# NVIDIA/tacotron2

Measured on AMD Instinct MI355X. Metric: mel-frames/sec (train fwd+bwd) LJSpeech hparams, higher is better.
Workload: dtype bf16; 1 GPU; BASELINE configs[1]: LJSpeech default hparams, batch_size=64/GPU, synthetic LJSpeech-shaped batches, full train step (fwd+loss+bwd+clip+Adam); global_batch=64, parallelism=dp1, optimizer=FusedAdam, compute=bf16 MFMA operands, f32 accumulate/state/master weights

## Files before the change

### include/tacotron2_amd.h

```cpp
#ifndef TACOTRON2_AMD_H
#define TACOTRON2_AMD_H

#include <stdint.h>

#ifdef __cplusplus
extern "C" {
#endif

#define T2AMD_ABI_VERSION 1
#define T2AMD_OK 0
#define T2AMD_ERR_ARG 1
#define T2AMD_ERR_LAUNCH 2

#define T2AMD_ATT_DIM 128
#define T2AMD_LOC_FILTERS 32
#define T2AMD_LOC_KERNEL 31
#define T2AMD_LOC_TAPS (2 * T2AMD_LOC_KERNEL)
#define T2AMD_ATT_SLICES 4

int t2amd_abi_version(void);
const char* t2amd_source_sha1(void);
const char* t2amd_last_error(void);
int t2amd_struct_sizes(int* out, int max_n);
int t2amd_set_validate_only(int on);
// ... 3 lines not shown

typedef struct t2amd_gemm_desc {
    const float* A;
    const float* B;
    float* C;
    int M, N, K;
    long long lda, ldb, ldc;
    int a_kcontig;
    int b_kcontig;
    int batch;
    long long strideA, strideB, strideC;
    int splitk;
    long long strideSplitC;
    int accumulate;
    const float* bias;
    int act;
    const uint8_t* keep;
    long long ldkeep;
    float keep_scale;
    int convA_T, convA_C, convA_pad, convA_sign;
    int convB_T, convB_C, convB_pad;
    int precision;
} t2amd_gemm_desc;

int t2amd_gemm_tile_size(int M, int N, int precision, int nz, int a_kcontig, int b_kcontig);
int t2amd_gemm_f32(const t2amd_gemm_desc* d, void* stream);

int t2amd_splitk_reduce_f32(const float* partials, int nsplit, long long stride, float* out,
                            long long n, int accumulate, int perm_taps, int perm_ci, void* stream);
int t2amd_splitk_reduce2d_f32(const float* partials, int nsplit, long long stride, float* out, int rows, int cols,
                              long long ldo, int accumulate, void* stream);

typedef struct t2amd_gemm16_desc {
    const void* A;
    const void* B;
    float* C;
    int M, N, K;
    long long lda, ldb, ldc;
    int splitk;
    long long strideSplitC;
    int accumulate;
    const float* bias;
    int win_T, win_Tp;
} t2amd_gemm16_desc;
int t2amd_gemm16_tn(const t2amd_gemm16_desc* d, void* stream);
int t2amd_gemm16_kk(const t2amd_gemm16_desc* d, void* stream);
// ... 653 lines not shown
```

### tacotron2_amd/csrc/attention.hip

```cpp
#include "common.h"
#include "cell_bwd.h"
#include "skinny_wide.h"
#include <vector>
#include <cstring>
#include <stdlib.h>
#include <stddef.h>

__device__ unsigned int t2_attn_timeouts = 0u;
__device__ __forceinline__ void t2_attn_gave_up() { atomicAdd(&t2_attn_timeouts, 1u); }
extern "C" int t2amd_attn_handoff_timeouts(int reset) {
    if (t2amd_validate_only_flag_()) return 0;
    unsigned int v = 0u;
    if (hipMemcpyFromSymbol(&v, HIP_SYMBOL(t2_attn_timeouts), sizeof(v)) != hipSuccess) return -1;
    if (reset && v != 0u) {
        const unsigned int z = 0u;
        (void)hipMemcpyToSymbol(HIP_SYMBOL(t2_attn_timeouts), &z, sizeof(z));
    }
    return (int)(v > 0x7fffffffu ? 0x7fffffffu : v);
}
__global__ void t2_attn_bump_kernel() { t2_attn_gave_up(); }
extern "C" int t2amd_debug_attn_timeout_(void* stream) {
    hipLaunchKernelGGL(t2_attn_bump_kernel, dim3(1), dim3(1), 0, (hipStream_t)stream);
    return hipGetLastError() == hipSuccess ? 0 : -1;
}
// ... 2435 lines not shown
extern "C" int t2amd_attention_step_bwd_f32(const t2amd_attn_bwd* a, void* stream) {
    return attn_bwd_step_impl(a, stream);
}


__global__ void fold_location_kernel(const float* __restrict__ wd, const float* __restrict__ wc,
                                     float* __restrict__ U) {
    const int i = blockIdx.x * blockDim.x + threadIdx.x;
    if (i < AD * NTAP) {
        const int d = i / NTAP, ck = i - d * NTAP;
        float s = 0.f;
        for (int f = 0; f < T2AMD_LOC_FILTERS; ++f) s = fmaf(wd[d * T2AMD_LOC_FILTERS + f], wc[f * NTAP + ck], s);
        U[i] = s;
    }
}

extern "C" int t2amd_fold_location_f32(const float* wdense, const float* wconv, float* U, void* stream) {
    T2_REQUIRE(wdense && wconv && U && t2_aligned16(U), "fold_location: bad pointers");
    T2_LAUNCH(fold_location_kernel, dim3((AD * NTAP + 255) / 256), dim3(256), 0, (hipStream_t)stream, wdense, wconv, U);
    T2_LAUNCH_CHECK();
    return T2AMD_OK;
}

__global__ __launch_bounds__(256) void unfold_location_reduce_kernel(const float* __restrict__ dU_acc, const float* __restrict__ dv_acc,
                                                                     int nb, float* __restrict__ dv, float* __restrict__ dUsum) {
    const int i = blockIdx.x * 256 + threadIdx.x;
    if (i < AD * NTAP) {
        float s = 0.f;
        int b = 0;
        for (; b + 8 <= nb; b += 8) {
            float v[8];
#pragma unroll
            for (int j = 0; j < 8; ++j) v[j] = dU_acc[(long long)(b + j) * AD * NTAP + i];
#pragma unroll
            for (int j = 0; j < 8; ++j) s += v[j];
        }
        for (; b < nb; ++b) s += dU_acc[(long long)b * AD * NTAP + i];
        dUsum[i] = s;
    } else if (i < AD * NTAP + AD) {
        const int d = i - AD * NTAP;
        float s = 0.f;
        for (int b = 0; b < nb; ++b) s += dv_acc[(long long)b * AD + d];
        dv[d] = s;
    }
}
__global__ __launch_bounds__(256) void unfold_location_products_kernel(const float* __restrict__ dUsum, const float* __restrict__ wd,
                                                                       const float* __restrict__ wc, float* __restrict__ dwd,
                                                                       float* __restrict__ dwc) {
    const int i = blockIdx.x * 256 + threadIdx.x;
    if (i < AD * T2AMD_LOC_FILTERS) {
        const int d = i / T2AMD_LOC_FILTERS, f = i - d * T2AMD_LOC_FILTERS;
        float s = 0.f;
        for (int ck = 0; ck < NTAP; ++ck) s = fmaf(dUsum[d * NTAP + ck], wc[f * NTAP + ck], s);
        dwd[i] = s;
    } else if (i < AD * T2AMD_LOC_FILTERS + T2AMD_LOC_FILTERS * NTAP) {
        const int o = i - AD * T2AMD_LOC_FILTERS;
        const int f = o / NTAP, ck = o - f * NTAP;
        float s = 0.f;
        for (int d = 0; d < AD; ++d) s = fmaf(wd[d * T2AMD_LOC_FILTERS + f], dUsum[d * NTAP + ck], s);
        dwc[o] = s;
    }
}

extern "C" int t2amd_unfold_location_grads_f32(const float* dU_acc, const float* dv_acc, int nb,
                                               const float* wdense, const float* wconv, float* dwdense,
                                               float* dwconv, float* dv, void* stream) {
    T2_REQUIRE(dU_acc && dv_acc && nb > 0 && wdense && wconv && dwdense && dwconv && dv, "unfold_location: bad args");
    float* dUsum = const_cast<float*>(dU_acc);
    T2_LAUNCH(unfold_location_reduce_kernel, dim3(t2_cdiv(AD * NTAP + AD, 256)), dim3(256), 0, (hipStream_t)stream, dU_acc, dv_acc, nb,
              dv, dUsum);
    T2_LAUNCH(unfold_location_products_kernel, dim3(t2_cdiv(AD * T2AMD_LOC_FILTERS + T2AMD_LOC_FILTERS * NTAP, 256)), dim3(256), 0,
              (hipStream_t)stream, dUsum, wdense, wconv, dwdense, dwconv);
    T2_LAUNCH_CHECK();
    return T2AMD_OK;
}
```

### tacotron2_amd/csrc/gemm.hip

```cpp
#include "common.h"

#define GBM 128
#define GBN 128
#define GBK 16
#define GLD 132

struct GemmParams {
    t2amd_gemm_desc d;
    int avec, bvec;
    int ktiles_per_split;
};

struct TileId { int bx, by, bz; };
__device__ __forceinline__ TileId xcd_tile_id() {
    const int nbx = gridDim.x, nby = gridDim.y;
    const int total = nbx * nby * (int)gridDim.z;
    const int L = blockIdx.x + nbx * (blockIdx.y + nby * blockIdx.z);
    const int xcd = L & 7, q = L >> 3;
    const int base = total >> 3, rem = total & 7;
    const int id = xcd * base + (xcd < rem ? xcd : rem) + q;
    const int per_z = nbx * nby;
    TileId t;
    t.bz = id / per_z;
    const int r = id - t.bz * per_z;
    const int G = 8;
    const int group = r / (G * nbx);
    const int first = group * G;
    const int gsz = (nby - first) < G ? (nby - first) : G;
    const int w = r - group * (G * nbx);
    t.by = first + w % gsz;
    t.bx = w / gsz;
    return t;
}
// ... 220 lines not shown
#pragma unroll
    for (int tm = 0; tm < 2; ++tm) {
#pragma unroll
        for (int tn = 0; tn < 2; ++tn) {
            const int gn = col0 + wn * 64 + tn * 32 + l31;
#pragma unroll
            for (int r = 0; r < 16; ++r) {
                const int row = (r & 3) + 8 * (r >> 2) + 4 * lhi;
                const int gm = row0 + wm * 64 + tm * 32 + row;
                if (gm < M && gn < N) {
                    float val = acc[tm][tn][r];
                    float* cp = C + (long long)gm * d.ldc + gn;
                    if (d.bias) val += d.bias[gn];
                    if (d.accumulate) val += *cp;
                    if (d.act == 1) val = fmaxf(val, 0.f);
                    if (d.keep) val = d.keep[(long long)gm * d.ldkeep + gn] ? val * d.keep_scale : 0.f;
                    *cp = val;
                }
            }
        }
    }
}

template <bool AK, bool BKC, bool X3, int TB>
__global__ __launch_bounds__(2 * TB) void gemm_bf16x3_kernel(GemmParams p);

extern "C" int t2amd_gemm_tile_size(int M, int N, int precision, int nz, int a_kcontig, int b_kcontig) {
    static const bool force128 = [] { const char* e = getenv("T2AMD_GEMM_TILE"); return e && atoi(e) == 128; }();
    if (force128 || precision < 1 || M < 512 || N < 512) return 128;
    if (precision == 1 && (a_kcontig || b_kcontig)) return 128;
    const long long wgs = (long long)t2_cdiv(M, 256) * t2_cdiv(N, 256) * (nz > 0 ? nz : 1);
    return wgs >= 192 ? 256 : 128;
}

extern "C" int t2amd_gemm_f32(const t2amd_gemm_desc* dp, void* stream) {
    T2_REQUIRE(dp != nullptr, "gemm: null descriptor");
    GemmParams p;
    p.d = *dp;
    t2amd_gemm_desc& d = p.d;
    T2_REQUIRE(d.A && d.B && d.C, "gemm: null operand");
    T2_REQUIRE(d.M > 0 && d.N > 0 && d.K >= 0, "gemm: bad dims");
    if (d.batch < 1) d.batch = 1;
    if (d.splitk < 1) d.splitk = 1;
    if (d.convA_T > 0) {
        T2_REQUIRE(d.a_kcontig == 1, "gemm: convA needs K-contiguous A");
        T2_REQUIRE(d.convA_C % GBK == 0 && d.K % d.convA_C == 0, "gemm: convA_C must be a multiple of 16 dividing K");
        T2_REQUIRE(d.convA_sign == 1 || d.convA_sign == -1, "gemm: convA_sign must be +-1");
        T2_REQUIRE(d.M % d.convA_T == 0, "gemm: convA rows must be whole utterances");
    }
    if (d.convB_T > 0) {
        T2_REQUIRE(d.b_kcontig == 0, "gemm: convB needs N-contiguous B");
        T2_REQUIRE(d.convB_C % 4 == 0 && d.N % d.convB_C == 0, "gemm: convB_C must be a multiple of 4 dividing N");
        T2_REQUIRE(d.K % d.convB_T == 0, "gemm: convB rows must be whole utterances");
    }
    if (d.splitk > 1) {
        T2_REQUIRE(!d.bias && !d.keep && d.act == 0 && !d.accumulate, "gemm: split-K needs a plain epilogue");
    }
    T2_REQUIRE(d.act == 0 || d.act == 1, "gemm: act must be 0 or 1");
    if (d.a_kcontig) {
        const int kdim = d.convA_T > 0 ? d.convA_C : d.K;
        p.avec = (kdim % 4 == 0) && (d.lda % 4 == 0) && t2_aligned16(d.A) && (d.strideA % 4 == 0);
    } else {
        p.avec = (d.M % 4 == 0) && (d.lda % 4 == 0) && t2_aligned16(d.A) && (d.strideA % 4 == 0);
    }
    if (d.b_kcontig) {
        p.bvec = (d.K % 4 == 0) && (d.ldb % 4 == 0) && t2_aligned16(d.B) && (d.strideB % 4 == 0);
    } else {
        const int ndim = d.convB_T > 0 ? d.convB_C : d.N;
        p.bvec = (ndim % 4 == 0) && (d.ldb % 4 == 0) && t2_aligned16(d.B) && (d.strideB % 4 == 0);
    }
    T2_REQUIRE(d.precision >= 0 && d.precision <= 2, "gemm: precision must be 0 (exact f32), 1 (split-bf16 x3) or 2 (bf16)");
    const bool fast = d.precision >= 1 && (d.convA_T == 0 || d.convA_C % 32 == 0);
    const int bk = fast ? 32 : GBK;
    const int nkt = t2_cdiv(d.K, bk);
    p.ktiles_per_split = t2_cdiv(nkt > 0 ? nkt : 1, d.splitk);
    dim3 grid(t2_cdiv(d.N, GBN), t2_cdiv(d.M, GBM), d.batch * d.splitk);
    T2_REQUIRE(grid.y <= 65535 && grid.z <= 65535, "gemm: grid too large");
    hipStream_t s = (hipStream_t)stream;
    if (fast && d.precision == 1 && t2amd_gemm_tile_size(d.M, d.N, 1, d.batch * d.splitk, d.a_kcontig, d.b_kcontig) == 256) {
        dim3 g2(t2_cdiv(d.N, 256), t2_cdiv(d.M, 256), d.batch * d.splitk);
        static bool attr_set = false;
        if (!attr_set && !t2amd_validate_only_flag_()) {
            (void)hipFuncSetAttribute((const void*)gemm_bf16x3_kernel<false, false, true, 256>,
                                      hipFuncAttributeMaxDynamicSharedMemorySize, 0);
            attr_set = true;
        }
        T2_LAUNCH((gemm_bf16x3_kernel<false, false, true, 256>), g2, dim3(512), 0, s, p);
        T2_LAUNCH_CHECK();
        return T2AMD_OK;
    }
    if (fast && d.precision == 1) {
        if (d.a_kcontig && d.b_kcontig)
            T2_LAUNCH((gemm_bf16x3_kernel<true, true, true, 128>), grid, dim3(256), 0, s, p);
        else if (d.a_kcontig && !d.b_kcontig)
            T2_LAUNCH((gemm_bf16x3_kernel<true, false, true, 128>), grid, dim3(256), 0, s, p);
        else if (!d.a_kcontig && d.b_kcontig)
            T2_LAUNCH((gemm_bf16x3_kernel<false, true, true, 128>), grid, dim3(256), 0, s, p);
        else
            T2_LAUNCH((gemm_bf16x3_kernel<false, false, true, 128>), grid, dim3(256), 0, s, p);
        T2_LAUNCH_CHECK();
        return T2AMD_OK;
    }
    if (fast && d.precision == 2 && t2amd_gemm_tile_size(d.M, d.N, 2, d.batch * d.splitk, d.a_kcontig, d.b_kcontig) == 256) {
        dim3 g2(t2_cdiv(d.N, 256), t2_cdiv(d.M, 256), d.batch * d.splitk);
        if (d.a_kcontig && d.b_kcontig)
            T2_LAUNCH((gemm_bf16x3_kernel<true, true, false, 256>), g2, dim3(512), 0, s, p);
        else if (d.a_kcontig && !d.b_kcontig)
            T2_LAUNCH((gemm_bf16x3_kernel<true, false, false, 256>), g2, dim3(512), 0, s, p);
        else if (!d.a_kcontig && d.b_kcontig)
            T2_LAUNCH((gemm_bf16x3_kernel<false, true, false, 256>), g2, dim3(512), 0, s, p);
        else
            T2_LAUNCH((gemm_bf16x3_kernel<false, false, false, 256>), g2, dim3(512), 0, s, p);
        T2_LAUNCH_CHECK();
        return T2AMD_OK;
    }
    if (fast) {
        if (d.a_kcontig && d.b_kcontig)
            T2_LAUNCH((gemm_bf16x3_kernel<true, true, false, 128>), grid, dim3(256), 0, s, p);
        else if (d.a_kcontig && !d.b_kcontig)
            T2_LAUNCH((gemm_bf16x3_kernel<true, false, false, 128>), grid, dim3(256), 0, s, p);
        else if (!d.a_kcontig && d.b_kcontig)
            T2_LAUNCH((gemm_bf16x3_kernel<false, true, false, 128>), grid, dim3(256), 0, s, p);
        else
            T2_LAUNCH((gemm_bf16x3_kernel<false, false, false, 128>), grid, dim3(256), 0, s, p);
        T2_LAUNCH_CHECK();
// ... 82 lines not shown
}

typedef short bf16x8 __attribute__((ext_vector_type(8)));

#define HBM_ 128
#define HBN_ 128
#define HBK_ 32
#define HLD_ 40

__device__ __forceinline__ unsigned cvt_pk_bf16(float a, float b) {
    unsigned r;
    asm("v_cvt_pk_bf16_f32 %0, %1, %2" : "=v"(r) : "v"(a), "v"(b));
    return r;
}
__device__ __forceinline__ void split4(float x0, float x1, float x2, float x3, uint2& hi, uint2& lo) {
    hi.x = cvt_pk_bf16(x0, x1);
    hi.y = cvt_pk_bf16(x2, x3);
    const float h0 = __uint_as_float(hi.x << 16), h1 = __uint_as_float(hi.x & 0xffff0000u);
    const float h2 = __uint_as_float(hi.y << 16), h3 = __uint_as_float(hi.y & 0xffff0000u);
    lo.x = cvt_pk_bf16(x0 - h0, x1 - h1);
    lo.y = cvt_pk_bf16(x2 - h2, x3 - h3);
}

template <bool AK, bool BKC, bool X3, int TB>
__global__ __launch_bounds__(2 * TB) void gemm_bf16x3_kernel(GemmParams p) {
    constexpr int NTHR = 2 * TB;
    constexpr int WN = TB / 64;
    constexpr int TM = TB / 64;
    constexpr int NH = X3 ? 2 : 1;
    constexpr int ALD = AK ? HLD_ : 32, BLD = BKC ? HLD_ : 32;
    constexpr int AIMG = TB * ALD, BIMG = TB * BLD;
    __shared__ __attribute__((aligned(16))) unsigned short As[2][NH * AIMG];
    __shared__ __attribute__((aligned(16))) unsigned short Bs[2][NH * BIMG];

    const t2amd_gemm_desc& d = p.d;
    const int tid = threadIdx.x;
    const int lane = tid & 63;
    const int wave = tid >> 6;
    const int wm = wave / WN, wn = wave % WN;

    const TileId tile = xcd_tile_id();
    const int z = tile.bz;
    const int bidx = z / d.splitk;
    const int split = z - bidx * d.splitk;
    const float* __restrict__ A = d.A + (long long)bidx * d.strideA;
    const float* __restrict__ B = d.B + (long long)bidx * d.strideB;
    float* __restrict__ C = d.C + (long long)bidx * d.strideC + (long long)split * d.strideSplitC;

    const int row0 = tile.by * TB;
    const int col0 = tile.bx * TB;
    const int M = d.M, N = d.N;
    const int kbeg = split * p.ktiles_per_split * HBK_;
    int kend = kbeg + p.ktiles_per_split * HBK_;
    if (kend > d.K) kend = d.K;
    const int nk = (kend > kbeg) ? (kend - kbeg + HBK_ - 1) / HBK_ : 0;

    int a_t[4] = {0, 0, 0, 0};
    if (AK && d.convA_T > 0) {
#pragma unroll
        for (int i = 0; i < 4; ++i) a_t[i] = (row0 + ((tid + NTHR * i) >> 3)) % d.convA_T;
    }
    int b_tap = 0, b_ci = 0;
    if (!BKC && d.convB_T > 0) {
        const int gn = col0 + (tid & (TB / 4 - 1)) * 4;
        b_tap = gn / d.convB_C;
        b_ci = gn - b_tap * d.convB_C;
    }

    float4 ra[4], rb[4];

    auto load_a = [&](int k0) {
#pragma unroll
        for (int i = 0; i < 4; ++i) {
            float4 v = make_float4(0.f, 0.f, 0.f, 0.f);
            if (AK) {
                const int f = tid + NTHR * i;
                const int r = f >> 3, kq = f & 7;
                const int gm = row0 + r;
                const int gk = k0 + kq * 4;
                if (gm < M && gk < kend) {
                    long long srow = gm;
                    int col = gk;
                    bool ok = true;
                    if (d.convA_T > 0) {
                        const int tap = k0 / d.convA_C;
                        col = (k0 - tap * d.convA_C) + kq * 4;
                        const int sh = (tap - d.convA_pad) * d.convA_sign;
                        const int tt = a_t[i] + sh;
                        ok = (tt >= 0) && (tt < d.convA_T);
                        srow = (long long)gm + sh;
                    }
                    if (ok) {
                        const float* src = A + srow * d.lda + col;
                        if (p.avec) {
// ... 7 lines not shown
                    }
                }
            } else {
                const int m4 = tid & (TB / 4 - 1), kq = tid / (TB / 4);
                const int gk = k0 + kq * 4 + i;
                const int gm = row0 + m4 * 4;
                if (gk < kend && gm < M) {
                    const float* src = A + (long long)gk * d.lda + gm;
                    if (p.avec) {
                        v = *reinterpret_cast<const float4*>(src);
                    } else {
                        v.x = src[0];
                        if (gm + 1 < M) v.y = src[1];
                        if (gm + 2 < M) v.z = src[2];
                        if (gm + 3 < M) v.w = src[3];
                    }
                }
            }
            ra[i] = v;
        }
    };

    auto load_b = [&](int k0) {
#pragma unroll
        for (int i = 0; i < 4; ++i) {
            float4 v = make_float4(0.f, 0.f, 0.f, 0.f);
            if (BKC) {
                const int f = tid + NTHR * i;
                const int r = f >> 3, kq = f & 7;
                const int gn = col0 + r;
                const int gk = k0 + kq * 4;
                if (gn < N && gk < kend) {
                    const float* src = B + (long long)gn * d.ldb + gk;
                    if (p.bvec) {
                        v = *reinterpret_cast<const float4*>(src);
                    } else {
                        v.x = src[0];
                        if (gk + 1 < kend) v.y = src[1];
                        if (gk + 2 < kend) v.z = src[2];
                        if (gk + 3 < kend) v.w = src[3];
                    }
                }
            } else {
                const int n4 = tid & (TB / 4 - 1), kq = tid / (TB / 4);
                const int gk = k0 + kq * 4 + i;
                const int gn = col0 + n4 * 4;
// ... 76 lines not shown
        } else {
            const unsigned* P = reinterpret_cast<const unsigned*>(S);
            const int p0 = ks * 8 + lhi_ * 4;
            union { unsigned u[4]; bf16x8 v; } t;
            t.u[0] = P[(p0 + 0) * TB + row];
            t.u[1] = P[(p0 + 1) * TB + row];
            t.u[2] = P[(p0 + 2) * TB + row];
            t.u[3] = P[(p0 + 3) * TB + row];
            return t.v;
        }
    };

    f32x16 acc[TM][2];
#pragma unroll
    for (int i = 0; i < TM; ++i)
#pragma unroll
        for (int j = 0; j < 2; ++j)
#pragma unroll
            for (int r = 0; r < 16; ++r) acc[i][j][r] = 0.f;

    if (nk > 0) {
        load_a(kbeg);
        load_b(kbeg);
        store_one(As[0], AIMG, AK, ra);
        store_one(Bs[0], BIMG, BKC, rb);
    }
    __syncthreads();

    const int l31 = lane & 31, lhi = lane >> 5;
    int cur = 0;
    for (int kt = 0; kt < nk; ++kt) {
        const bool more = (kt + 1 < nk);
        if (more) {
            load_a(kbeg + (kt + 1) * HBK_);
            load_b(kbeg + (kt + 1) * HBK_);
        }
#pragma unroll
        for (int ks = 0; ks < HBK_ / 16; ++ks) {
            bf16x8 ah[TM], al[TM], bh[2], bl[2];
#pragma unroll
            for (int t = 0; t < TM; ++t) {
                ah[t] = frag(As[cur], AK, wm * (32 * TM) + t * 32 + l31, ks, lhi);
                if (X3) al[t] = frag(As[cur] + AIMG, AK, wm * (32 * TM) + t * 32 + l31, ks, lhi);
            }
#pragma unroll
            for (int t = 0; t < 2; ++t) {
                bh[t] = frag(Bs[cur], BKC, wn * 64 + t * 32 + l31, ks, lhi);
                if (X3) bl[t] = frag(Bs[cur] + BIMG, BKC, wn * 64 + t * 32 + l31, ks, lhi);
            }
#pragma unroll
            for (int i = 0; i < TM; ++i)
#pragma unroll
                for (int j = 0; j < 2; ++j) {
                    if (X3) {
                        acc[i][j] = __builtin_amdgcn_mfma_f32_32x32x16_bf16(al[i], bh[j], acc[i][j], 0, 0, 0);
                        acc[i][j] = __builtin_amdgcn_mfma_f32_32x32x16_bf16(ah[i], bl[j], acc[i][j], 0, 0, 0);
                    }
                    acc[i][j] = __builtin_amdgcn_mfma_f32_32x32x16_bf16(ah[i], bh[j], acc[i][j], 0, 0, 0);
                }
        }
        if (more) {
            store_one(As[cur ^ 1], AIMG, AK, ra);
            store_one(Bs[cur ^ 1], BIMG, BKC, rb);
        }
        __syncthreads();
        cur ^= 1;
    }

#pragma unroll
    for (int tm = 0; tm < TM; ++tm) {
#pragma unroll
        for (int tn = 0; tn < 2; ++tn) {
            const int gn = col0 + wn * 64 + tn * 32 + l31;
#pragma unroll
            for (int r = 0; r < 16; ++r) {
                const int row = (r & 3) + 8 * (r >> 2) + 4 * lhi;
                const int gm = row0 + wm * (32 * TM) + tm * 32 + row;
                if (gm < M && gn < N) {
                    float val = acc[tm][tn][r];
                    float* cp = C + (long long)gm * d.ldc + gn;
                    if (d.bias) val += d.bias[gn];
                    if (d.accumulate) val += *cp;
                    if (d.act == 1) val = fmaxf(val, 0.f);
                    if (d.keep) val = d.keep[(long long)gm * d.ldkeep + gn] ? val * d.keep_scale : 0.f;
                    *cp = val;
                }
// ... 5 lines not shown
```

### tacotron2_amd/csrc/rnn.hip

```cpp
#include "common.h"
#include "cell_bwd.h"
#include <hip/hip_ext.h>

#include "skinny_wide.h"

#define SK_DEPTH 4

template <bool LSTM, int TAG, bool BF>
__global__ __launch_bounds__(256) void skinny_gemm_kernel(SkinnyDual dp) {
    constexpr int ES = BF ? 2 : 4;
    constexpr int BK = 256 / ES;
    constexpr int EPC = 16 / ES;
    __shared__ __attribute__((aligned(16))) float smem[SK_NBUF * (SK_XT + SK_WT) + SK_ROWS * 17];
    float* const Xs = smem;
    float* const Ws = smem + SK_NBUF * SK_XT;
    float* const Os = smem + SK_NBUF * (SK_XT + SK_WT);

    const bool second = (int)blockIdx.x >= dp.nblk0;
    const SkinnyParams p = skinny_select(dp, second);
    const int lb = (int)blockIdx.x - (second ? dp.nblk0 : 0);
    const int bx = lb % p.gx;
    const int by = (lb / p.gx) % p.gy;
    const int bz = lb / (p.gx * p.gy);

// ... 550 lines not shown
    }
}

static bool skinny_wide_enabled() {
    static const bool on = [] { const char* e = getenv("T2AMD_SKINNY_NARROW"); return !(e && e[0] == '1'); }();
    return on;
}

static inline int sk_bk(int mode) { return (mode == 1 || mode == 2) ? 128 : 64; }
static int check_segs(const t2amd_seg* x, int nseg, int Ktot, int bk) {
    if (nseg < 1 || nseg > 3) T2_FAIL("skinny: nseg must be 1..3");
    int sum = 0;
    for (int i = 0; i < nseg; ++i) {
        if (x[i].width <= 0 || x[i].width % bk != 0) T2_FAIL("skinny: segment widths must be positive multiples of 64 (f32, split-bf16 x3) / 128 (bf16)");
        if (x[i].p && (!t2_aligned16(x[i].p) || x[i].ld % 8 != 0)) T2_FAIL("skinny: segment must be 16-byte aligned with ld % 8 == 0");
        sum += x[i].width;
    }
    if (sum != Ktot) T2_FAIL("skinny: segment widths do not add up to Ktot");
    return T2AMD_OK;
}

static int fill_lstm(const t2amd_lstm_step* a, SkinnyParams& p) {
    T2_REQUIRE(a != nullptr, "lstm_step: null args");
    T2_REQUIRE(a->bf16 >= 0 && a->bf16 <= 3, "lstm_step: bf16 must be 0 (f32), 1 (bf16), 2 (bf16 weights only, small batch) or 3 (split-bf16 x3)");
    T2_PROPAGATE(check_segs(a->x, a->nseg, a->Ktot, sk_bk(a->bf16)));
    T2_REQUIRE(a->W && t2_aligned16(a->W), "lstm_step: W must be 16-byte aligned");
    T2_REQUIRE(a->H > 0 && a->H % 4 == 0 && a->B > 0, "lstm_step: H must be a multiple of 4");
    T2_REQUIRE(a->c_out && a->h_out, "lstm_step: null outputs");
    p = SkinnyParams{};
    for (int i = 0; i < 3; ++i) p.x[i] = a->x[i];
    p.nseg = a->nseg;
    p.W = a->W; p.Ktot = a->Ktot; p.B = a->B; p.H = a->H; p.N = 4 * a->H;
    p.gin = a->gin; p.ld_gin = a->ld_gin; p.bias = a->bias;
    p.c_prev = a->c_prev; p.ld_cprev = a->ld_cprev;
    p.gates_out = a->gates_out; p.ld_gates = a->ld_gates;
    p.c_out = a->c_out; p.ld_c = a->ld_c; p.h_out = a->h_out; p.ld_h = a->ld_h;
    p.h16_out = (unsigned short*)a->h16_out; p.ld_h16 = a->ld_h16;
    p.keep = a->keep; p.ld_keep = a->ld_keep; p.keep_scale = a->keep_scale;
    p.lens = a->lens; p.t = a->t;
    p.gx = a->H / 4; p.gy = t2_cdiv(a->B, SK_ROWS); p.gz = 1;
    p.wcol[0] = p.wcol[1] = p.wcol[2] = -1;
    return T2AMD_OK;
}

static int lstm_step_fwd2_impl(const t2amd_lstm_step* a, const t2amd_lstm_step* b, int swap01, void* stream) {
    SkinnyDual d;
    d.ts = t2amd_debug_ts_();
// ... 266 lines not shown
```

### tacotron2_amd/engine.py

```python
import os

import math
import torch

from . import native as nv
from .native import NativeError

BN_EPS = 1e-5
BN_MOMENTUM = 0.1


def check_hparams(hp):
    if hp.n_frames_per_step != 1:
        raise ValueError("n_frames_per_step != 1 is not supported (nor by the reference, hparams.py:56)")
    K = hp.attention_location_kernel_size
    if not (1 <= hp.attention_dim <= nv.ATT_DIM and 1 <= hp.attention_location_n_filters <= nv.LOC_FILTERS
            and 1 <= K <= nv.LOC_KERNEL and K % 2 == 1):
        raise ValueError("the attention kernels hold attention_dim <= %d, <= %d location filters and an odd location "
                         "kernel <= %d (smaller geometries run zero-embedded in the compiled one; an even kernel size "
                         "does not run in the reference either: ConvNorm pads (k-1)//2, model.py:18-20)"
                         % (nv.ATT_DIM, nv.LOC_FILTERS, nv.LOC_KERNEL))
    for name in ('encoder_embedding_dim', 'attention_rnn_dim', 'decoder_rnn_dim', 'prenet_dim'):
        if getattr(hp, name) % 64 != 0:
            raise ValueError("%s must be a multiple of 64 for the MFMA recurrent kernels" % name)
# ... 189 lines not shown
    except ValueError:
        ns = -1
    if not 1 <= ns <= 8:
        raise NativeError("T2AMD_DGRAD_SPLIT must be an integer in 1..8, got %r" % (raw,))
    return ns


DGRAD_SPLIT = _dgrad_split()


def _enc_dgrad_split():
    raw = os.environ.get('T2AMD_ENC_DGRAD_SPLIT', '4')
    if raw not in ('1', '2', '4'):
        raise NativeError("T2AMD_ENC_DGRAD_SPLIT must be 1, 2 or 4, got %r" % (raw,))
    return int(raw)


ENC_DGRAD_SPLIT = _enc_dgrad_split()

BN_BWD_IMAGE = os.environ.get('T2AMD_BN_BWD_IMAGE', '1') != '0'
BN_FWD_IMAGE = os.environ.get('T2AMD_BN_FWD_IMAGE', '1') != '0'
BIAS_GRAD16 = os.environ.get('T2AMD_BIAS_GRAD16', '1') != '0'
GATE_GRADS_BF16_ONLY = os.environ.get('T2AMD_GATE_GRADS_BF16_ONLY', '1') != '0'
DXD_RING = int(os.environ.get('T2AMD_DXD_RING', '3'))


def _rg(run, *a, **k):
    return run.gemm(*a, fast=run.gradp, **k)


def _ng(run, *a, **k):
    return nv.gemm(*a, fast=run.gradp, **k)


def _fg(run, *a, exact=False, **k):
    return nv.gemm(*a, fast=(0 if (exact and run.x3) else run.fwdp), **k)


_PACK_GEN = [0]


def bump_weight_generation():
    _PACK_GEN[0] += 1


ARENA = os.environ.get('T2AMD_ARENA', '1') != '0'
# ... 820 lines not shown
                      HA16=run.empty16(To, B, Ha),
                      HD16=run.empty16(To, B, Hd), CTX16=run.empty16(To, B, E), memory16=run.cast16(memory),
                      Wq16=run.cached('Wq16', [Wq], lambda: run.cast16(Wq)))
        d.bf16 = 1
        for k_, v_ in c.bf16.items():
            setattr(d, k_, nv.ptr(v_, torch.bfloat16))
    elif run.x3:
        c.bf16 = dict(Wa_rec16=run.cached('Wa_rec16x3', [Wih_a, Whh_a], lambda: run.split16(Wa_rec)),
                      Wd_cat16=run.cached('Wd_cat16x3', [Wih_d, Whh_d], lambda: run.split16(Wd_cat)),
                      HA16=run.empty16(To, B, 2 * Ha), HD16=run.empty16(To, B, 2 * Hd), CTX16=run.empty16(To, B, 2 * E))
        d.bf16 = 3
        for k_, v_ in c.bf16.items():
            setattr(d, k_, nv.ptr(v_, torch.bfloat16))
    op16 = run.bf16 or run.x3
    model.last_train_decoder_path = _decoder_train_fwd(
        model, run, d, poison=slabs['CTX'] if training else None,
        reads=[Wa_rec, Wd_cat, bias_d, Wq, U, vvec, memory, pm, lens32, keep_att, keep_dec]
        + ([c.bf16[k_] for k_ in ('Wa_rec16', 'Wd_cat16')] if op16 else []) + ([c.bf16[k_] for k_ in ('memory16', 'Wq16')] if run.bf16 else []),
        writes=[GA] + list(slabs.values()) + ([c.bf16[k_] for k_ in ('HA16', 'HD16', 'CTX16')] if op16 else []),
        regen_ga=project_ga)

    Wpg, bpg = _packed_projection(run, P, Cm, Hd, E)
    PG = run.empty(rowsD, Cm + 1)
    _fg(run, PG, slabs['HD'].view(rowsD, Hd), Wpg[:, :Hd])
    _fg(run, PG, slabs['CTX'].view(rowsD, E), Wpg[:, Hd:], accumulate=True, bias=bpg)
    mel_cl = run.empty(B, To, Cm)
    gate = run.out_empty(B, To)
    nv.split_projection(PG, mel_cl, gate, olens32)

    npost = hp.postnet_n_convolutions
    rowsP = B * To
    post_chans = [hp.postnet_embedding_dim] * (npost - 1) + [Cm]
    post_masks = [ms.get('post', i, (B, To, post_chans[i]), 0.5) for i in range(npost)] if training else None
    post_cl, c.post_saved = _conv_stack_fwd(run, P, bufs, 'postnet.convolutions', npost,
                                            mel_cl.view(rowsP, Cm), To, [2] * (npost - 1) + [0],
                                            post_masks, training)
    mel = run.out_empty(B, Cm, To)
    mel_post = run.out_empty(B, Cm, To)
    nv.finalize_outputs(mel_cl, post_cl.view(B, To, Cm), mel, mel_post, olens32)

    c.run = run
    c.dec = d
    c.keep = dict(att=keep_att, dec=keep_dec, k0=k0, k1=k1)
    c.slabs = slabs
    c.tensors = dict(x0=x0, p1=p1, p2=p2, pm=pm, GA=GA, Wa_rec=Wa_rec, Wd_cat=Wd_cat, bias_d=bias_d,
                     Wq=Wq, U=U, Wpg=Wpg, mel_cl=mel_cl, vvec=vvec, lens32=lens32)
    return (mel, mel_post, gate, slabs['ALIGN']), c
# ... 28 lines not shown
        G_own, staged = G, {}

        def G(name, *shape):
            if name in embedded:
                staged[name] = run.empty(*shape)
                return staged[name]
            return G_own(name, *shape)

    dmel_cl = run.empty(B, To, Cm)
    dpost_cl = run.empty(B, To, Cm)
    nv.grads_to_channel_last(cont(d_mel), cont(d_post), dmel_cl, dpost_cl)
    _conv_stack_bwd(run, P, g, 'postnet.convolutions', c.post_saved, dpost_cl.view(rowsP, Cm), To,
                    first_dx=dmel_cl.view(rowsP, Cm), first_dx_accumulate=True, G=G)
    if sync is not None:
        sync.bucket_ready('postnet')
    dout = run.empty(rowsD, Cm + 1)
    nv.gather_dout(dmel_cl, cont(d_gate), dout)

    Wpg = T['Wpg']
    DHC = run.empty(rowsD, Hd + E)
    _ng(run, DHC, dout, Wpg, b_kn=True)
    dWpg_h = run.empty(Cm + 1, Hd)
    dWpg_c = run.empty(Cm + 1, E)
    _rg(run, dWpg_h, dout, S['HD'].view(rowsD, Hd), a_km=True, b_kn=True)
    _rg(run, dWpg_c, dout, S['CTX'].view(rowsD, E), a_km=True, b_kn=True)
    dWp = G('decoder.linear_projection.linear_layer.weight', Cm, Hd + E)
    dWg = G('decoder.gate_layer.linear_layer.weight', 1, Hd + E)
    nv.copy2d(dWp[:, :Hd], dWpg_h[:Cm]); nv.copy2d(dWp[:, Hd:], dWpg_c[:Cm])
    nv.copy2d(dWg[:, :Hd], dWpg_h[Cm:]); nv.copy2d(dWg[:, Hd:], dWpg_c[Cm:])
    dbpg = run.empty(Cm + 1)
    run.colsum(dout, dbpg)
    dbp = G('decoder.linear_projection.linear_layer.bias', Cm)
    dbg = G('decoder.gate_layer.linear_layer.bias', 1)
    nv.copy2d(dbp.view(1, Cm), dbpg[:Cm].view(1, Cm))
    nv.copy2d(dbg.view(1, 1), dbpg[Cm:].view(1, 1))
    g['decoder.linear_projection.linear_layer.weight'] = dWp
    g['decoder.gate_layer.linear_layer.weight'] = dWg
    g['decoder.linear_projection.linear_layer.bias'] = dbp
    g['decoder.gate_layer.linear_layer.bias'] = dbg

    Wq = P['decoder.attention_layer.query_layer.linear_layer.weight']
    Wih_a, Whh_a = P['decoder.attention_rnn.weight_ih'], P['decoder.attention_rnn.weight_hh']
    Wih_d, Whh_d = P['decoder.decoder_rnn.weight_ih'], P['decoder.decoder_rnn.weight_hh']

    def transposed(src, rows, cols):
        Wt = run.empty(rows, cols)
        nv.transpose(Wt, src)
        return Wt
# ... 34 lines not shown
        for k_, v_ in b16.items():
            setattr(bw, k_, nv.ptr(v_, torch.bfloat16))
    op16 = run.bf16 or run.x3
    model.last_train_decoder_bwd_path = _decoder_train_bwd(model, run, bw, out['dv_acc'],
                              reads=[Wa_recT, Wd_catT, DHC, cont(d_align), T['Wq'], T['U'], T['vvec'], T['pm'], c.memory,
                                     T['lens32'], T['GA'], c.keep['att'], c.keep['dec']]
                              + [S[k_] for k_ in ('HA', 'CA', 'GD', 'HD', 'CD', 'CTX', 'Q', 'ALIGN', 'CUM')]
                              + ([b16['Wa_recT16'], b16['Wd_catT16']] if op16 else [])
                              + ([c.bf16['memory16'], c.bf16['Wq16']] if run.bf16 else []),
                              writes=[v_ for v_ in out.values() if v_ is not None] + [S['attn_ws']] + ([b16['DGA16'], b16['DGD16']] if op16 else []))
    DGA, DGD, DCTX, DQ, d_pm = (out[k_] for k_ in ('DGA', 'DGD', 'DCTX', 'DQ', 'd_pm'))
    DGA2, DGD2 = (None, None) if drop32 else (DGA.view(rowsD, 4 * Ha), DGD.view(rowsD, 4 * Hd))

    Wdense = P['decoder.attention_layer.location_layer.location_dense.linear_layer.weight']
    Wconv = P['decoder.attention_layer.location_layer.location_conv.conv.weight']
    dWdense = G('decoder.attention_layer.location_layer.location_dense.linear_layer.weight', A, nv.LOC_FILTERS)
    dWconv = G('decoder.attention_layer.location_layer.location_conv.conv.weight', nv.LOC_FILTERS, 2, nv.LOC_KERNEL)
    dv = G('decoder.attention_layer.v.linear_layer.weight', 1, A)
    nv.unfold_location_grads(out['dU_acc'], out['dv_acc'], B, Wdense, Wconv, dWdense, dWconv, dv)
    g['decoder.attention_layer.location_layer.location_dense.linear_layer.weight'] = dWdense
    g['decoder.attention_layer.location_layer.location_conv.conv.weight'] = dWconv
    g['decoder.attention_layer.v.linear_layer.weight'] = dv
    dWq = G('decoder.attention_layer.query_layer.linear_layer.weight', A, Ha)
    _rg(run, dWq, DQ.view(rowsD, A), S['HA'].view(rowsD, Ha), a_km=True, b_kn=True)
    g['decoder.attention_layer.query_layer.linear_layer.weight'] = dWq

    dWih_a = G('decoder.attention_rnn.weight_ih', 4 * Ha, Pd + E)
    dWhh_a = G('decoder.attention_rnn.weight_hh', 4 * Ha, Ha)
    use16 = run.bf16 and WGRAD16 and B % 8 == 0 and not nv.validate_only()
    Z = c.bf16 if use16 else None
    if use16:
        _lstm_wgrad16(run, b16['DGA16'].view(rowsD, 4 * Ha), B, [(T['p2'], False), (Z['CTX16'].view(rowsD, E), True), (Z['HA16'].view(rowsD, Ha), True)],
                      [(dWih_a, 0, 2), (dWhh_a, 2, 3)])
    elif To > 1:
        tmp = run.empty(4 * Ha, Pd)
        _rg(run, tmp, DGA2, T['p2'], a_km=True, b_kn=True)
        nv.copy2d(dWih_a[:, :Pd], tmp)
        sh = (To - 1) * B
        tmp2 = run.empty(4 * Ha, E)
        _rg(run, tmp2, DGA2[B:], S['CTX'].view(rowsD, E)[:sh], a_km=True, b_kn=True)
        nv.copy2d(dWih_a[:, Pd:], tmp2)
        _rg(run, dWhh_a, DGA2[B:], S['HA'].view(rowsD, Ha)[:sh], a_km=True, b_kn=True)
    else:
        tmp = run.empty(4 * Ha, Pd)
        _rg(run, tmp, DGA2, T['p2'], a_km=True, b_kn=True)
        nv.copy2d(dWih_a[:, :Pd], tmp)
        nv.fill(dWhh_a, 0.0)
# ... 619 lines not shown
```

### tacotron2_amd/native.py

```python
import ctypes as C
import os

import torch

_HERE = os.path.dirname(os.path.abspath(__file__))
LIB_PATH = os.environ.get("T2AMD_LIB", os.path.join(_HERE, "lib", "libtacotron2_amd.so"))

TORCH_OPS_PATH = os.path.join(_HERE, "lib", "libtacotron2_amd_torch.so")

ATT_DIM = 128
LOC_FILTERS = 32
LOC_KERNEL = 31
LOC_TAPS = 62
ATT_SLICES = 4

_f32p = C.c_void_p
_i64 = C.c_longlong


class GemmDesc(C.Structure):
    _fields_ = [
        ("A", _f32p), ("B", _f32p), ("C", _f32p),
        ("M", C.c_int), ("N", C.c_int), ("K", C.c_int),
        ("lda", _i64), ("ldb", _i64), ("ldc", _i64),
# ... 647 lines not shown
    if dtype is not None and t.dtype != dtype:
        raise NativeError("tacotron2_amd: expected %s, got %s" % (dtype, t.dtype))
    return C.c_void_p(t.data_ptr())


def _mat(t, dtype=torch.float32):
    if t.dim() != 2 or (t.shape[1] > 1 and t.stride(1) != 1):
        raise NativeError("expected a 2-D tensor with contiguous rows, got shape %s stride %s"
                          % (tuple(t.shape), t.stride()))
    ld = t.stride(0) if t.shape[0] > 1 else max(t.stride(0), t.shape[1])
    return ptr(t, dtype), ld, t.shape[0], t.shape[1]


def _fullc(t):
    if not t.is_contiguous():
        raise NativeError("expected a contiguous tensor, got shape %s stride %s" % (tuple(t.shape), t.stride()))
    return t


def scale_for(p):
    return float(torch.tensor(1.0, dtype=torch.float32) / torch.tensor(1.0 - p, dtype=torch.float32))


def gemm_tile_size(M, N, precision, nz=1, a_km=False, b_kn=False):
    return int(load().t2amd_gemm_tile_size(int(M), int(N), int(precision), int(nz), 0 if a_km else 1, 0 if b_kn else 1))


def gemm(Cm, A, B, a_km=False, b_kn=False, accumulate=False, bias=None, act=0, keep=None,
         keep_scale=1.0, convA=None, convB=None, batch=1, strides=(0, 0, 0), splitk=1, partials=None,
         fast=False):
    lib = load()
    d = GemmDesc()
    pa, lda, r0, c0 = _mat(A)
    pb, ldb, r1, c1 = _mat(B)
    pc, ldc, M, N = _mat(Cm)
    Ka, Ma = (r0, c0) if a_km else (c0, r0)
    Kb, Nb = (r1, c1) if b_kn else (c1, r1)
    if convA is not None:
        if a_km or Ka != convA[1] or Kb % convA[1] != 0:
            raise NativeError("gemm: convA needs A=[rows,C] and K(B) a multiple of C")
        K = Kb
    else:
        K = Ka
    if convB is not None:
        if not b_kn or Nb != convB[1] or N % convB[1] != 0:
            raise NativeError("gemm: convB needs B=[rows,C] (b_kn) and N(C) a multiple of C")
        Nb = N
    if Ma != M or Nb != N or Kb != K:
        raise NativeError("gemm: shape mismatch C=%s A=%s B=%s (a_km=%s b_kn=%s K=%d)"
                          % (tuple(Cm.shape), tuple(A.shape), tuple(B.shape), a_km, b_kn, K))
    d.A, d.B, d.C = pa, pb, pc
    d.M, d.N, d.K = M, N, K
    d.lda, d.ldb, d.ldc = lda, ldb, ldc
    d.a_kcontig = 0 if a_km else 1
    d.b_kcontig = 0 if b_kn else 1
    d.batch = batch
    d.strideA, d.strideB, d.strideC = strides
    d.splitk = splitk
    d.precision = int(fast)
    d.accumulate = 1 if accumulate else 0
    d.bias = ptr(bias)
    d.act = act
    if keep is not None:
        if keep.dim() != 2 or tuple(keep.shape) != (M, N) or keep.stride(1) != 1:
            raise NativeError("gemm: keep mask must be a [M,N] uint8 view, got %s" % (tuple(keep.shape),))
        d.keep, d.ldkeep, d.keep_scale = ptr(keep, torch.uint8), keep.stride(0), keep_scale
    if convA is not None:
        d.convA_T, d.convA_C, d.convA_pad, d.convA_sign = convA
    if convB is not None:
        d.convB_T, d.convB_C, d.convB_pad = convB
    if splitk > 1:
        if partials is None or partials.numel() < splitk * M * N or not partials.is_contiguous():
            raise NativeError("gemm: split-K needs a contiguous partials buffer")
        d.C = ptr(partials)
        d.ldc = N
        d.strideSplitC = M * N
    _check(lib.t2amd_gemm_f32(C.byref(d), _stream()), "t2amd_gemm_f32")


def gemm16_tn(Cm, A16, B16, K=None, splitk=1, partials=None, accumulate=False, bias=None):
    lib = load()
    d = Gemm16Desc()
# ... 1631 lines not shown
```

Measured before the change: 648,500 valid mel-frames/s.

## Let the bf16 GEMM read one operand directly from its bf16 image

Adds flag bits so the generic GEMM can take one operand that is already stored as bf16. The kernel then loads eight bf16 values per vector and writes them straight into shared memory, without reading f32 and converting. The decoder projection forward and backward and the query-weight gradient now read the existing HD16, CTX16 and HA16 bf16 copies instead of the f32 slabs, which halves operand read traffic. It also fixes pointer constness in the location-unfold reduce and tightens the LSTM bf16 mode check. The cost is a new kernel template variant, and the new path always uses the 128-tile kernel rather than the 256-tile path.

```diff
diff --git a/include/tacotron2_amd.h b/include/tacotron2_amd.h
--- a/include/tacotron2_amd.h
+++ b/include/tacotron2_amd.h
@@ -49,6 +49,8 @@
     int convB_T, convB_C, convB_pad;
     int precision;
 } t2amd_gemm_desc;
+#define T2AMD_GEMM_A_BF16 0x10
+#define T2AMD_GEMM_B_BF16 0x20
 
 int t2amd_gemm_tile_size(int M, int N, int precision, int nz, int a_kcontig, int b_kcontig);
 int t2amd_gemm_f32(const t2amd_gemm_desc* d, void* stream);
diff --git a/tacotron2_amd/csrc/attention.hip b/tacotron2_amd/csrc/attention.hip
--- a/tacotron2_amd/csrc/attention.hip
+++ b/tacotron2_amd/csrc/attention.hip
@@ -2481,8 +2481,8 @@
     return T2AMD_OK;
 }
 
-__global__ __launch_bounds__(256) void unfold_location_reduce_kernel(const float* __restrict__ dU_acc, const float* __restrict__ dv_acc,
-                                                                     int nb, float* __restrict__ dv, float* __restrict__ dUsum) {
+__global__ __launch_bounds__(256) void unfold_location_reduce_kernel(float* dU_acc, const float* __restrict__ dv_acc,
+                                                                     int nb, float* __restrict__ dv, float* dUsum) {
     const int i = blockIdx.x * 256 + threadIdx.x;
     if (i < AD * NTAP) {
         float s = 0.f;
@@ -2526,7 +2526,7 @@
                                                float* dwconv, float* dv, void* stream) {
     T2_REQUIRE(dU_acc && dv_acc && nb > 0 && wdense && wconv && dwdense && dwconv && dv, "unfold_location: bad args");
     float* dUsum = const_cast<float*>(dU_acc);
-    T2_LAUNCH(unfold_location_reduce_kernel, dim3(t2_cdiv(AD * NTAP + AD, 256)), dim3(256), 0, (hipStream_t)stream, dU_acc, dv_acc, nb,
+    T2_LAUNCH(unfold_location_reduce_kernel, dim3(t2_cdiv(AD * NTAP + AD, 256)), dim3(256), 0, (hipStream_t)stream, dUsum, dv_acc, nb,
               dv, dUsum);
     T2_LAUNCH(unfold_location_products_kernel, dim3(t2_cdiv(AD * T2AMD_LOC_FILTERS + T2AMD_LOC_FILTERS * NTAP, 256)), dim3(256), 0,
               (hipStream_t)stream, dUsum, wdense, wconv, dwdense, dwconv);
diff --git a/tacotron2_amd/csrc/gemm.hip b/tacotron2_amd/csrc/gemm.hip
--- a/tacotron2_amd/csrc/gemm.hip
+++ b/tacotron2_amd/csrc/gemm.hip
@@ -9,6 +9,7 @@
     t2amd_gemm_desc d;
     int avec, bvec;
     int ktiles_per_split;
+    int a16, b16;
 };
 
 struct TileId { int bx, by, bz; };
@@ -275,7 +276,7 @@
     }
 }
 
-template <bool AK, bool BKC, bool X3, int TB>
+template <bool AK, bool BKC, bool X3, int TB, int S16 = 0>
 __global__ __launch_bounds__(2 * TB) void gemm_bf16x3_kernel(GemmParams p);
 
 extern "C" int t2amd_gemm_tile_size(int M, int N, int precision, int nz, int a_kcontig, int b_kcontig) {
@@ -310,17 +311,26 @@
         T2_REQUIRE(!d.bias && !d.keep && d.act == 0 && !d.accumulate, "gemm: split-K needs a plain epilogue");
     }
     T2_REQUIRE(d.act == 0 || d.act == 1, "gemm: act must be 0 or 1");
+    p.a16 = (d.precision & T2AMD_GEMM_A_BF16) ? 1 : 0;
+    p.b16 = (d.precision & T2AMD_GEMM_B_BF16) ? 1 : 0;
+    d.precision &= ~(T2AMD_GEMM_A_BF16 | T2AMD_GEMM_B_BF16);
+    if (p.a16 || p.b16) {
+        T2_REQUIRE(d.precision == 2, "gemm: a bf16-image operand needs the plain bf16 product (precision 2)");
+        T2_REQUIRE(!(p.a16 && p.b16), "gemm: at most one bf16-image operand (two belong on t2amd_gemm16_tn / _kk)");
+        T2_REQUIRE(d.convA_T == 0 && d.convB_T == 0, "gemm: no implicit convolution over a bf16-image operand");
+    }
+    const int va = p.a16 ? 8 : 4, vb = p.b16 ? 8 : 4;
     if (d.a_kcontig) {
         const int kdim = d.convA_T > 0 ? d.convA_C : d.K;
-        p.avec = (kdim % 4 == 0) && (d.lda % 4 == 0) && t2_aligned16(d.A) && (d.strideA % 4 == 0);
+        p.avec = (kdim % va == 0) && (d.lda % va == 0) && t2_aligned16(d.A) && (d.strideA % va == 0);
     } else {
-        p.avec = (d.M % 4 == 0) && (d.lda % 4 == 0) && t2_aligned16(d.A) && (d.strideA % 4 == 0);
+        p.avec = (d.M % va == 0) && (d.lda % va == 0) && t2_aligned16(d.A) && (d.strideA % va == 0);
     }
     if (d.b_kcontig) {
-        p.bvec = (d.K % 4 == 0) && (d.ldb % 4 == 0) && t2_aligned16(d.B) && (d.strideB % 4 == 0);
+        p.bvec = (d.K % vb == 0) && (d.ldb % vb == 0) && t2_aligned16(d.B) && (d.strideB % vb == 0);
     } else {
         const int ndim = d.convB_T > 0 ? d.convB_C : d.N;
-        p.bvec = (ndim % 4 == 0) && (d.ldb % 4 == 0) && t2_aligned16(d.B) && (d.strideB % 4 == 0);
+        p.bvec = (ndim % vb == 0) && (d.ldb % vb == 0) && t2_aligned16(d.B) && (d.strideB % vb == 0);
     }
     T2_REQUIRE(d.precision >= 0 && d.precision <= 2, "gemm: precision must be 0 (exact f32), 1 (split-bf16 x3) or 2 (bf16)");
     const bool fast = d.precision >= 1 && (d.convA_T == 0 || d.convA_C % 32 == 0);
@@ -354,6 +364,23 @@
         T2_LAUNCH_CHECK();
         return T2AMD_OK;
     }
+    if (p.a16 || p.b16) {
+#define T2_GEMM_SRC16(S)                                                                                          \
+        do {                                                                                                      \
+            if (d.a_kcontig && d.b_kcontig)                                                                       \
+                T2_LAUNCH((gemm_bf16x3_kernel<true, true, false, 128, S>), grid, dim3(256), 0, s, p);             \
+            else if (d.a_kcontig && !d.b_kcontig)                                                                 \
+                T2_LAUNCH((gemm_bf16x3_kernel<true, false, false, 128, S>), grid, dim3(256), 0, s, p);            \
+            else if (!d.a_kcontig && d.b_kcontig)                                                                 \
+                T2_LAUNCH((gemm_bf16x3_kernel<false, true, false, 128, S>), grid, dim3(256), 0, s, p);            \
+            else                                                                                                  \
+                T2_LAUNCH((gemm_bf16x3_kernel<false, false, false, 128, S>), grid, dim3(256), 0, s, p);           \
+        } while (0)
+        if (p.a16) T2_GEMM_SRC16(1); else T2_GEMM_SRC16(2);
+#undef T2_GEMM_SRC16
+        T2_LAUNCH_CHECK();
+        return T2AMD_OK;
+    }
     if (fast && d.precision == 2 && t2amd_gemm_tile_size(d.M, d.N, 2, d.batch * d.splitk, d.a_kcontig, d.b_kcontig) == 256) {
         dim3 g2(t2_cdiv(d.N, 256), t2_cdiv(d.M, 256), d.batch * d.splitk);
         if (d.a_kcontig && d.b_kcontig)
@@ -482,8 +509,18 @@
     lo.y = cvt_pk_bf16(x2 - h2, x3 - h3);
 }
 
-template <bool AK, bool BKC, bool X3, int TB>
+__device__ __forceinline__ uint4 load8_bf16(const unsigned short* src, bool vec, int n) {
+    if (vec) return *reinterpret_cast<const uint4*>(src);
+    unsigned u[4] = {0u, 0u, 0u, 0u};
+#pragma unroll
+    for (int j = 0; j < 8; ++j)
+        if (j < n) u[j >> 1] |= (unsigned)src[j] << ((j & 1) * 16);
+    return make_uint4(u[0], u[1], u[2], u[3]);
+}
+
+template <bool AK, bool BKC, bool X3, int TB, int S16>
 __global__ __launch_bounds__(2 * TB) void gemm_bf16x3_kernel(GemmParams p) {
+    static_assert(S16 == 0 || !X3, "a bf16 image has no lo half");
     constexpr int NTHR = 2 * TB;
     constexpr int WN = TB / 64;
     constexpr int TM = TB / 64;
@@ -503,8 +540,10 @@
     const int z = tile.bz;
     const int bidx = z / d.splitk;
     const int split = z - bidx * d.splitk;
-    const float* __restrict__ A = d.A + (long long)bidx * d.strideA;
-    const float* __restrict__ B = d.B + (long long)bidx * d.strideB;
+    const float* __restrict__ A = d.A + ((S16 & 1) ? 0 : (long long)bidx * d.strideA);
+    const float* __restrict__ B = d.B + ((S16 & 2) ? 0 : (long long)bidx * d.strideB);
+    const unsigned short* __restrict__ A16 = reinterpret_cast<const unsigned short*>(d.A) + (long long)bidx * d.strideA;
+    const unsigned short* __restrict__ B16 = reinterpret_cast<const unsigned short*>(d.B) + (long long)bidx * d.strideB;
     float* __restrict__ C = d.C + (long long)bidx * d.strideC + (long long)split * d.strideSplitC;
 
     const int row0 = tile.by * TB;
@@ -528,8 +567,46 @@
     }
 
     float4 ra[4], rb[4];
+    uint4 qa[2], qb[2];
+
+    auto load_img = [&](uint4 (&q)[2], const unsigned short* P, long long ld, bool vec, bool kc, int r0, int rlim, int k0) {
+#pragma unroll
+        for (int i = 0; i < 2; ++i) {
+            uint4 v = make_uint4(0u, 0u, 0u, 0u);
+            if (kc) {
+                const int f = tid + NTHR * i;
+                const int g = r0 + (f >> 2), gk = k0 + (f & 3) * 8;
+                if (g < rlim && gk < kend) v = load8_bf16(P + (long long)g * ld + gk, vec, kend - gk);
+            } else {
+                const int g = r0 + (tid % (TB / 8)) * 8, gk = k0 + (tid / (TB / 8)) * 2 + i;
+                if (g < rlim && gk < kend) v = load8_bf16(P + (long long)gk * ld + g, vec, rlim - g);
+            }
+            q[i] = v;
+        }
+    };
+    auto store_img = [&](unsigned short* S, bool kc, const uint4 (&q)[2]) {
+        if (kc) {
+#pragma unroll
+            for (int i = 0; i < 2; ++i) {
+                const int f = tid + NTHR * i;
+                *reinterpret_cast<uint4*>(&S[(f >> 2) * HLD_ + (f & 3) * 8]) = q[i];
+            }
+        } else {
+            unsigned* Pp = reinterpret_cast<unsigned*>(S) + (tid / (TB / 8)) * TB + (tid % (TB / 8)) * 8;
+            const unsigned e[4] = {q[0].x, q[0].y, q[0].z, q[0].w}, o[4] = {q[1].x, q[1].y, q[1].z, q[1].w};
+            unsigned w[8];
+#pragma unroll
+            for (int j = 0; j < 4; ++j) {
+                w[2 * j] = (e[j] & 0xffffu) | (o[j] << 16);
+                w[2 * j + 1] = (e[j] >> 16) | (o[j] & 0xffff0000u);
+            }
+            *reinterpret_cast<uint4*>(Pp) = make_uint4(w[0], w[1], w[2], w[3]);
+            *reinterpret_cast<uint4*>(Pp + 4) = make_uint4(w[4], w[5], w[6], w[7]);
+        }
+    };
 
     auto load_a = [&](int k0) {
+        if (S16 & 1) { load_img(qa, A16, d.lda, p.avec, AK, row0, M, k0); return; }
 #pragma unroll
         for (int i = 0; i < 4; ++i) {
             float4 v = make_float4(0.f, 0.f, 0.f, 0.f);
@@ -583,6 +660,7 @@
     };
 
     auto load_b = [&](int k0) {
+        if (S16 & 2) { load_img(qb, B16, d.ldb, p.bvec, BKC, col0, N, k0); return; }
 #pragma unroll
         for (int i = 0; i < 4; ++i) {
             float4 v = make_float4(0.f, 0.f, 0.f, 0.f);
@@ -705,8 +783,8 @@
     if (nk > 0) {
         load_a(kbeg);
         load_b(kbeg);
-        store_one(As[0], AIMG, AK, ra);
-        store_one(Bs[0], BIMG, BKC, rb);
+        if (S16 & 1) store_img(As[0], AK, qa); else store_one(As[0], AIMG, AK, ra);
+        if (S16 & 2) store_img(Bs[0], BKC, qb); else store_one(Bs[0], BIMG, BKC, rb);
     }
     __syncthreads();
 
@@ -743,8 +821,8 @@
                 }
         }
         if (more) {
-            store_one(As[cur ^ 1], AIMG, AK, ra);
-            store_one(Bs[cur ^ 1], BIMG, BKC, rb);
+            if (S16 & 1) store_img(As[cur ^ 1], AK, qa); else store_one(As[cur ^ 1], AIMG, AK, ra);
+            if (S16 & 2) store_img(Bs[cur ^ 1], BKC, qb); else store_one(Bs[cur ^ 1], BIMG, BKC, rb);
         }
         __syncthreads();
         cur ^= 1;
diff --git a/tacotron2_amd/csrc/rnn.hip b/tacotron2_amd/csrc/rnn.hip
--- a/tacotron2_amd/csrc/rnn.hip
+++ b/tacotron2_amd/csrc/rnn.hip
@@ -596,7 +596,7 @@
 
 static int fill_lstm(const t2amd_lstm_step* a, SkinnyParams& p) {
     T2_REQUIRE(a != nullptr, "lstm_step: null args");
-    T2_REQUIRE(a->bf16 >= 0 && a->bf16 <= 3, "lstm_step: bf16 must be 0 (f32), 1 (bf16), 2 (bf16 weights only, small batch) or 3 (split-bf16 x3)");
+    T2_REQUIRE(a->bf16 == 0 || a->bf16 == 1 || a->bf16 == 3, "lstm_step: bf16 must be 0 (f32), 1 (bf16) or 3 (split-bf16 x3)");
     T2_PROPAGATE(check_segs(a->x, a->nseg, a->Ktot, sk_bk(a->bf16)));
     T2_REQUIRE(a->W && t2_aligned16(a->W), "lstm_step: W must be 16-byte aligned");
     T2_REQUIRE(a->H > 0 && a->H % 4 == 0 && a->B > 0, "lstm_step: H must be a multiple of 4");
diff --git a/tacotron2_amd/engine.py b/tacotron2_amd/engine.py
--- a/tacotron2_amd/engine.py
+++ b/tacotron2_amd/engine.py
@@ -235,6 +235,7 @@
 BN_FWD_IMAGE = os.environ.get('T2AMD_BN_FWD_IMAGE', '1') != '0'
 BIAS_GRAD16 = os.environ.get('T2AMD_BIAS_GRAD16', '1') != '0'
 GATE_GRADS_BF16_ONLY = os.environ.get('T2AMD_GATE_GRADS_BF16_ONLY', '1') != '0'
+GEMM_SRC16 = os.environ.get('T2AMD_GEMM_SRC16', '1') != '0'
 DXD_RING = int(os.environ.get('T2AMD_DXD_RING', '3'))
 
 
@@ -1101,7 +1102,8 @@
 
     Wpg, bpg = _packed_projection(run, P, Cm, Hd, E)
     PG = run.empty(rowsD, Cm + 1)
-    _fg(run, PG, slabs['HD'].view(rowsD, Hd), Wpg[:, :Hd])
+    src16 = run.bf16 and GEMM_SRC16
+    _fg(run, PG, (c.bf16['HD16'] if src16 else slabs['HD']).view(rowsD, Hd), Wpg[:, :Hd])
     _fg(run, PG, slabs['CTX'].view(rowsD, E), Wpg[:, Hd:], accumulate=True, bias=bpg)
     mel_cl = run.empty(B, To, Cm)
     gate = run.out_empty(B, To)
@@ -1176,8 +1178,9 @@
     _ng(run, DHC, dout, Wpg, b_kn=True)
     dWpg_h = run.empty(Cm + 1, Hd)
     dWpg_c = run.empty(Cm + 1, E)
-    _rg(run, dWpg_h, dout, S['HD'].view(rowsD, Hd), a_km=True, b_kn=True)
-    _rg(run, dWpg_c, dout, S['CTX'].view(rowsD, E), a_km=True, b_kn=True)
+    src16 = run.bf16 and GEMM_SRC16
+    _rg(run, dWpg_h, dout, (c.bf16['HD16'] if src16 else S['HD']).view(rowsD, Hd), a_km=True, b_kn=True)
+    _rg(run, dWpg_c, dout, (c.bf16['CTX16'] if src16 else S['CTX']).view(rowsD, E), a_km=True, b_kn=True)
     dWp = G('decoder.linear_projection.linear_layer.weight', Cm, Hd + E)
     dWg = G('decoder.gate_layer.linear_layer.weight', 1, Hd + E)
     nv.copy2d(dWp[:, :Hd], dWpg_h[:Cm]); nv.copy2d(dWp[:, Hd:], dWpg_c[:Cm])
@@ -1258,7 +1261,7 @@
     g['decoder.attention_layer.location_layer.location_conv.conv.weight'] = dWconv
     g['decoder.attention_layer.v.linear_layer.weight'] = dv
     dWq = G('decoder.attention_layer.query_layer.linear_layer.weight', A, Ha)
-    _rg(run, dWq, DQ.view(rowsD, A), S['HA'].view(rowsD, Ha), a_km=True, b_kn=True)
+    _rg(run, dWq, DQ.view(rowsD, A), (c.bf16['HA16'] if src16 else S['HA']).view(rowsD, Ha), a_km=True, b_kn=True)
     g['decoder.attention_layer.query_layer.linear_layer.weight'] = dWq
 
     dWih_a = G('decoder.attention_rnn.weight_ih', 4 * Ha, Pd + E)
diff --git a/tacotron2_amd/native.py b/tacotron2_amd/native.py
--- a/tacotron2_amd/native.py
+++ b/tacotron2_amd/native.py
@@ -693,6 +693,9 @@
     return float(torch.tensor(1.0, dtype=torch.float32) / torch.tensor(1.0 - p, dtype=torch.float32))
 
 
+GEMM_A_BF16, GEMM_B_BF16 = 0x10, 0x20
+
+
 def gemm_tile_size(M, N, precision, nz=1, a_km=False, b_kn=False):
     return int(load().t2amd_gemm_tile_size(int(M), int(N), int(precision), int(nz), 0 if a_km else 1, 0 if b_kn else 1))
 
@@ -702,8 +705,11 @@
          fast=False):
     lib = load()
     d = GemmDesc()
-    pa, lda, r0, c0 = _mat(A)
-    pb, ldb, r1, c1 = _mat(B)
+    a16, b16 = A.dtype == torch.bfloat16, B.dtype == torch.bfloat16
+    if (a16 or b16) and (int(fast) != 2 or (a16 and b16) or convA is not None or convB is not None):
+        raise NativeError("gemm: a bf16-image operand needs fast=2, f32 for the other operand and no convolution")
+    pa, lda, r0, c0 = _mat(A, A.dtype if a16 else torch.float32)
+    pb, ldb, r1, c1 = _mat(B, B.dtype if b16 else torch.float32)
     pc, ldc, M, N = _mat(Cm)
     Ka, Ma = (r0, c0) if a_km else (c0, r0)
     Kb, Nb = (r1, c1) if b_kn else (c1, r1)
@@ -728,7 +734,7 @@
     d.batch = batch
     d.strideA, d.strideB, d.strideC = strides
     d.splitk = splitk
-    d.precision = int(fast)
+    d.precision = int(fast) | (GEMM_A_BF16 if a16 else 0) | (GEMM_B_BF16 if b16 else 0)
     d.accumulate = 1 if accumulate else 0
     d.bias = ptr(bias)
     d.act = act
```

After: 649,800 valid mel-frames/s, median of 2. About the same (+0.2%).
